# themattinthehatt/behavenet

Measured on AMD Instinct MI355X. Metric: AE training frames/sec (128x128x1, batch 256), higher is better.
Workload: dtype f32; 1 GPU; configs[1]: conv AE default arch, 1x128x128 f32 frames resident in HBM, 12 latents, batch 256 (chunks 200+56), fwd+bwd+Adam(amsgrad)

## Files before the change

behavenet_amd/csrc/conv_mfma_up.hip:

```cpp
#include <stdlib.h>
#include "bn_common.h"
#include "bn_fast.h"
#ifndef UP2_ST_AUX
#define UP2_ST_AUX 2
#endif
#ifndef UP2_ST_AUX_D
#define UP2_ST_AUX_D UP2_ST_AUX
#endif


typedef float floatx16 __attribute__((ext_vector_type(16)));

#define MF_THREADS 256
#define MF_MAX_LDS (64 * 1024)

static inline int ilog2_exact_up(int v) {
    int l = 0;
    while ((1 << l) < v) ++l;
    return ((1 << l) == v) ? l : -1;
}

struct UpTile {
    int F, AT_H, lgW, lgATW;
    int SWp, FS, CHS;
    int tiles_per_frame;
    int xl_floats;
};

template <int MR, int CC>
__global__ __launch_bounds__(MF_THREADS, 2) void k_up_mfma(
    const float* __restrict__ small, const float* __restrict__ w, const float* __restrict__ bias,
    float* __restrict__ out, const float* __restrict__ dact_src, BnGeom g, UpTile t, int act,
    int dact, float slope) {
    extern __shared__ __attribute__((aligned(16))) float smem[];
    float* xl = smem;
    float* wl = smem + t.xl_floats;
    constexpr int RS = 25;
    constexpr int TM = 32 * MR;
    constexpr int WCH = TM * RS;
    constexpr int WGRP = CC * WCH / 4;
    constexpr int WDMA = (WGRP + MF_THREADS - 1) / MF_THREADS;
    constexpr int WBUF = ((WDMA * MF_THREADS * 4) + 3) & ~3;
    const int tid = threadIdx.x, lane = tid & 63;
    const int wv = __builtin_amdgcn_readfirstlane(tid >> 6);
    const int li = lane & 31, kk = lane >> 5;

    const int grp = blockIdx.x / t.tiles_per_frame;
    const int rowt = blockIdx.x - grp * t.tiles_per_frame;
    const int n0 = grp * t.F;
    const int a0 = rowt * t.AT_H;
    const int m0 = blockIdx.y * TM;
    const int Ws = g.Ws, HWs = g.Hs * g.Ws;

    const int pos = 32 * wv + li;
    const int pf = pos >> t.lgATW;
    const int prem = pos & ((1 << t.lgATW) - 1);
    const int aj = prem >> t.lgW, bj = prem & (Ws - 1);
    const int base = pf * t.FS + (aj + 1) * t.SWp + (bj + 1) + kk * t.CHS;
    const bool pvalid = (n0 + pf) < g.N;

    int ioff = -2;
    if (tid < t.CHS) {
        const int f = tid / t.FS;
        const int r2 = tid - f * t.FS;
        const int y = r2 / t.SWp;
        const int x = r2 - y * t.SWp;
        const int p = a0 - 1 + y, q = x - 1;
        const bool ok = (n0 + f < g.N) && p >= 0 && p < g.Hs && q >= 0 && q < g.Ws;
        ioff = ok ? f * (g.Cs * HWs) + p * Ws + q : -1;
    }

    floatx16 acc[MR][4];
#pragma unroll
    for (int mr = 0; mr < MR; ++mr)
#pragma unroll
        for (int cl = 0; cl < 4; ++cl)
#pragma unroll
            for (int e = 0; e < 16; ++e) acc[mr][cl][e] = 0.f;

    float xr[CC];
    const __amdgpu_buffer_rsrc_t rs_w = __builtin_amdgcn_make_buffer_rsrc(
        (void*)w, 0, (int)((size_t)g.Cs * g.Cb * RS * 4), 0x00020000);

    auto issue_loads = [&](int c0, int buf) {
#pragma unroll
        for (int cc = 0; cc < CC; ++cc) {
            const int c = min(c0 + cc, g.Cs - 1);
            xr[cc] = small[((size_t)n0 * g.Cs + c) * HWs + max(ioff, 0)];
        }
#pragma unroll
        for (int k = 0; k < WDMA; ++k) {
            const int e = tid + MF_THREADS * k;
            const int cc = e / (WCH / 4);
            const int within = e - cc * (WCH / 4);
            const bool ok = (e < WGRP) && (c0 + cc < g.Cs);
            const int off = (((c0 + cc) * g.Cb + m0) * RS + 4 * within) * 4;
            __builtin_amdgcn_raw_ptr_buffer_load_lds(
                rs_w, wl + buf * WBUF + 4 * (MF_THREADS * k + 64 * wv), 16, ok ? off : 0x7fffffff,
                0, 0, 0);
        }
    };

    int cur = 0;
    issue_loads(0, 0);
    for (int c0 = 0; c0 < g.Cs; c0 += CC) {
        __syncthreads();
#pragma unroll
        for (int cc = 0; cc < CC; ++cc) {
            const bool cok = c0 + cc < g.Cs;
            if (ioff != -2) xl[cc * t.CHS + tid] = (cok && ioff >= 0) ? xr[cc] : 0.f;
        }
        asm volatile("s_waitcnt vmcnt(0)" ::: "memory");
        __syncthreads();
        if (c0 + CC < g.Cs) issue_loads(c0 + CC, cur ^ 1);
        const float* wcur = wl + cur * WBUF;

#pragma unroll 1
        for (int cp = 0; cp < CC / 2; ++cp) {
            const float* xb = xl + (2 * cp) * t.CHS + base;
            const float* wa = wcur + ((2 * cp + kk) * TM + li) * RS;
            float bv[3][3];
#pragma unroll
            for (int dy = 0; dy < 3; ++dy)
#pragma unroll
                for (int dx = 0; dx < 3; ++dx) bv[dy][dx] = xb[(dy - 1) * t.SWp + (dx - 1)];
#pragma unroll
            for (int rho = 0; rho < 2; ++rho) {
#pragma unroll
                for (int u = 0; u < 3; ++u) {
                    const int r = ((rho + 1) & 1) + 2 * u;
                    if (r >= 5) continue;
                    const int dy = ((rho + 1) >> 1) - u + 1;
#pragma unroll
                    for (int sig = 0; sig < 2; ++sig) {
#pragma unroll
                        for (int v = 0; v < 3; ++v) {
                            const int s = ((sig + 1) & 1) + 2 * v;
                            if (s >= 5) continue;
                            const int dx = ((sig + 1) >> 1) - v + 1;
#pragma unroll
                            for (int mr = 0; mr < MR; ++mr) {
                                const float av = wa[mr * 32 * RS + r * 5 + s];
                                acc[mr][rho * 2 + sig] = __builtin_amdgcn_mfma_f32_32x32x2f32(
                                    av, bv[dy][dx], acc[mr][rho * 2 + sig], 0, 0, 0);
                            }
                        }
                    }
                }
            }
        }
        cur ^= 1;
    }

    if (!pvalid) return;
    const int n = n0 + pf;
    const int Wb = g.Wb, HWb = g.Hb * g.Wb;
    const int h0 = 2 * (a0 + aj), w0 = 2 * bj;
#pragma unroll
    for (int mr = 0; mr < MR; ++mr) {
#pragma unroll
        for (int e = 0; e < 16; ++e) {
            const int m = m0 + mr * 32 + (e & 3) + 8 * (e >> 2) + 4 * kk;
            if (m >= g.Cb) continue;
            const float bm = bias ? bias[m] : 0.f;
#pragma unroll
            for (int rho = 0; rho < 2; ++rho) {
                const size_t idx = ((size_t)n * g.Cb + m) * HWb + (size_t)(h0 + rho) * Wb + w0;
                float2 v;
                v.x = bn_apply_act(acc[mr][rho * 2 + 0][e] + bm, act, slope);
                v.y = bn_apply_act(acc[mr][rho * 2 + 1][e] + bm, act, slope);
                if (dact_src) {
                    const float2 d = *reinterpret_cast<const float2*>(dact_src + idx);
                    v.x *= bn_act_grad_from_output(d.x, dact, slope);
                    v.y *= bn_act_grad_from_output(d.y, dact, slope);
                }
                *reinterpret_cast<float2*>(out + idx) = v;
            }
        }
    }
}

#define UP2_STR2(x) #x
#define UP2_STR(x) UP2_STR2(x)
#ifndef UP2_LOOP_ALIGN
#define UP2_LOOP_ALIGN 8
#endif
#ifndef UP2_LOOP_SHIFT
#define UP2_LOOP_SHIFT 32
#endif
#ifndef UP2_WGS
#define UP2_WGS 2
#endif
template <int LGW>
struct UP2 {
    static constexpr int Ws = 1 << LGW, HW = Ws * Ws, TP = 128;
    static constexpr int F = HW >= TP ? 1 : TP / HW;
    static constexpr int AT_H = HW >= TP ? TP / Ws : Ws;
    static constexpr int lgATW = (HW >= TP) ? 7 : 2 * LGW;
    static constexpr int SWp = Ws + 2, FS = (AT_H + 2) * SWp, CHS = F * FS;
    static constexpr int CHSP = (CHS + 63) / 64 * 64;
    static constexpr int TPF = (F == 1) ? Ws / AT_H : 1;
};

template <>
struct UP2<0> {
    static constexpr int CHSP = 256;
};
template <>
struct UP2<1> {
    static constexpr int CHSP = 320;
};
struct Up2Geo {
    int F, AT_H, ATW;
    int SWp, FS, CHS;
    int UPF;
};

__device__ __forceinline__ void up_dma16(__amdgpu_buffer_rsrc_t rsrc, float* lds, int voffset, int soffset) {
    __builtin_amdgcn_raw_ptr_buffer_load_lds(rsrc, lds, 16, voffset, soffset, 0, 0);
}
__device__ __forceinline__ void up_dma4(__amdgpu_buffer_rsrc_t rsrc, float* lds, int voffset, int soffset) {
    __builtin_amdgcn_raw_ptr_buffer_load_lds(rsrc, lds, 4, voffset, soffset, 0, 0);
}

template <int KV>
__device__ __forceinline__ constexpr bool up2_tap_live(int r, int s) {
    return r >= KV / 10 && r < KV % 10 && s >= KV / 10 && s < KV % 10;
}

template <int LGW, int CC, int KV>
__global__ __launch_bounds__(MF_THREADS, UP2_WGS) void k_up2_mfma(
    const float* __restrict__ small, const float* __restrict__ w, const float* __restrict__ bias,
    float* __restrict__ out, const float* __restrict__ dact_src, BnGeom g, int act, int dact,
    float slope, int cper, size_t zstride, Up2Geo tg) {
    extern __shared__ __attribute__((aligned(16))) float smem[];
    using T = UP2<LGW>;
    constexpr bool RT = LGW <= 1;
    const int c_beg = blockIdx.z * cper;
    const int c_end = min(g.Cs, c_beg + cper);
    out += blockIdx.z * zstride;
    constexpr int RS = 25, TM = 32;
    const int Ws = RT ? g.Ws : (1 << LGW), HWs = RT ? g.Hs * g.Ws : (1 << (2 * LGW)), SWp = RT ? tg.SWp : Ws + 2;
    constexpr int XBUF = CC * T::CHSP;
    constexpr int WCH = TM * RS;
    constexpr int WGRP = CC * WCH / 4;
    constexpr int WDMA = (WGRP + MF_THREADS - 1) / MF_THREADS;
    constexpr int WBUF = WDMA * MF_THREADS * 4;
    constexpr int XW = T::CHSP > MF_THREADS ? MF_THREADS / 64 : T::CHSP / 64;
    constexpr int OOB = 0x7fffffff;
    const int tid = threadIdx.x, lane = tid & 63;
    const int wv = __builtin_amdgcn_readfirstlane(tid >> 6);
    const int li = lane & 31, kk = lane >> 5;

    int grp, rowt, n0, a0, pf, aj, bj, tFS, tCHS;
    bool pvalid;
    const int m0 = blockIdx.y * TM;
    int u0 = 0, lidx = 0;
    if constexpr (RT) {
        grp = rowt = 0;
        u0 = blockIdx.x * tg.F;
        n0 = u0 / tg.UPF;
        int pos = 32 * wv + li;
        const bool inside = pos < tg.F * tg.ATW;
        if (!inside) pos = 0;
        const int uf = pos / tg.ATW;
        const int prem = pos - uf * tg.ATW;
        const int un = (u0 + uf) / tg.UPF;
        a0 = (u0 + uf - un * tg.UPF) * tg.AT_H;
        aj = prem / Ws;
        bj = prem - aj * Ws;
        pvalid = inside && un < g.N && (a0 + aj) < g.Hs;
        pf = un - n0;
        tFS = tg.FS; tCHS = tg.CHS;
        lidx = uf;
    } else {
        grp = blockIdx.x / T::TPF;
        rowt = blockIdx.x - grp * T::TPF;
        n0 = grp * T::F;
        a0 = rowt * T::AT_H;
        const int pos = 32 * wv + li;
        pf = pos >> T::lgATW;
        const int prem = pos & ((1 << T::lgATW) - 1);
        aj = prem >> LGW; bj = prem & (Ws - 1);
        pvalid = (n0 + pf) < g.N;
        tFS = T::FS; tCHS = T::CHS;
        lidx = pf;
    }
    const int Hs_rt = RT ? g.Hs : Ws;

    const __amdgpu_buffer_rsrc_t rs_x = __builtin_amdgcn_make_buffer_rsrc(
        (void*)small, 0, (int)((size_t)g.N * g.Cs * HWs * 4), 0x00020000);
    const __amdgpu_buffer_rsrc_t rs_w = __builtin_amdgcn_make_buffer_rsrc(
        (void*)w, 0, (int)((size_t)g.Cs * g.Cb * RS * 4), 0x00020000);
    auto tile_elem = [&](const int el) {
        if (el >= tCHS) return OOB;
        const int f = el / tFS, r2 = el - f * tFS;
        const int y = r2 / SWp, x = r2 - y * SWp;
        int fn = f, fa0 = a0;
        if constexpr (RT) {
            const int un = (u0 + f) / tg.UPF;
            fn = un - n0;
            fa0 = (u0 + f - un * tg.UPF) * tg.AT_H;
        }
        const int p = fa0 - 1 + y, q = x - 1;
        const bool ok = (n0 + fn < g.N) && p >= 0 && p < Hs_rt && q >= 0 && q < Ws;
        return ok ? (fn * (g.Cs * HWs) + p * Ws + q) * 4 : OOB;
    };
    const int xvo = tile_elem(tid);
    constexpr int NX2 = T::CHSP > MF_THREADS ? CC : 0;
    int xvo2 = OOB;
    if constexpr (NX2 > 0) xvo2 = tile_elem(tid + MF_THREADS);
    int wvo[WDMA];
#pragma unroll
    for (int k = 0; k < WDMA; ++k) {
        const int e = tid + MF_THREADS * k;
        const int cc = e / (WCH / 4), within = e - cc * (WCH / 4);
        wvo[k] = (e < WGRP) ? ((cc * g.Cb + m0) * RS + 4 * within) * 4 : OOB;
    }
    auto issue_dma = [&](const int d, const int buf, const int c0) __attribute__((always_inline)) {
        if (d < CC) {
            if (wv < XW)
                up_dma4(rs_x, smem + buf * XBUF + d * T::CHSP + 64 * wv, xvo,
                        (n0 * g.Cs + c0 + d) * HWs * 4);
        } else if (d < CC + NX2) {
            if (wv == 0 && tCHS > MF_THREADS)
                up_dma4(rs_x, smem + buf * XBUF + (d - CC) * T::CHSP + MF_THREADS, xvo2,
                        (n0 * g.Cs + c0 + d - CC) * HWs * 4);
        } else {
            const int k = d - CC - NX2;
            up_dma16(rs_w, smem + 2 * XBUF + buf * WBUF + 4 * (MF_THREADS * k + 64 * wv), wvo[k],
                     c0 * g.Cb * RS * 4);
        }
    };
    constexpr int NDMA = CC + NX2 + WDMA;

    floatx16 acc[4];
#pragma unroll
    for (int cl = 0; cl < 4; ++cl)
#pragma unroll
        for (int e = 0; e < 16; ++e) acc[cl][e] = 0.f;

    int xb_cur = (lidx * tFS + (aj + 1) * SWp + (bj + 1) + kk * T::CHSP) * 4;
    int xb_oth = xb_cur + XBUF * 4;
    int wa_cur = (2 * XBUF + (kk * TM + li) * RS) * 4;
    int wa_oth = wa_cur + WBUF * 4;
    asm volatile("" : "+v"(xb_cur)); asm volatile("" : "+v"(xb_oth));
    asm volatile("" : "+v"(wa_cur)); asm volatile("" : "+v"(wa_oth));
    int xu_cur = xb_cur - SWp * 4, xd_cur = xb_cur + SWp * 4;
    int xu_oth = xb_oth - SWp * 4, xd_oth = xb_oth + SWp * 4;
    if constexpr (RT) {
        asm volatile("" : "+v"(xu_cur)); asm volatile("" : "+v"(xd_cur));
        asm volatile("" : "+v"(xu_oth)); asm volatile("" : "+v"(xd_oth));
    }
    const char* sm = reinterpret_cast<const char*>(smem);

    struct Tap { int r, s, dy, dx, cl; };
    auto tap_of = [](const int j) {
        int n = 0;
        Tap tp = {0, 0, 0, 0, 0};
        for (int rho = 0; rho < 2; ++rho)
            for (int u = 0; u < 3; ++u) {
                const int r = ((rho + 1) & 1) + 2 * u;
                if (r >= 5) continue;
                for (int sig = 0; sig < 2; ++sig)
                    for (int v = 0; v < 3; ++v) {
                        const int s = ((sig + 1) & 1) + 2 * v;
                        if (s >= 5) continue;
                        if (n == j) tp = Tap{r, s, ((rho + 1) >> 1) - u + 1, ((sig + 1) >> 1) - v + 1, rho * 2 + sig};
                        ++n;
                    }
            }
        return tp;
    };
    constexpr int ORDER[25] = {12, 10, 13, 2, 14, 11, 17, 3, 18, 15, 19, 4, 0, 22, 16, 7, 1, 23, 20, 8, 5, 24, 21, 9, 6};
    auto load_a = [&](const int wa, const int cp, const int jj, float (&a)[25]) __attribute__((always_inline)) {
        const int j = ORDER[jj];
        const Tap tp = tap_of(j);
        a[j] = *reinterpret_cast<const float*>(sm + wa + ((2 * cp) * TM * RS + tp.r * 5 + tp.s) * 4);
    };
    auto load_b = [&](const int xb, const int xu, const int xd, const int cp, const int i, float (&b)[9]) __attribute__((always_inline)) {
        const int dy = i / 3, dx = i - 3 * dy;
        if constexpr (RT) {
            const int xr = dy == 0 ? xu : dy == 1 ? xb : xd;
            b[i] = *reinterpret_cast<const float*>(sm + xr + ((2 * cp) * T::CHSP + (dx - 1)) * 4);
        } else {
            constexpr int SW = (1 << LGW) + 2;
            b[i] = *reinterpret_cast<const float*>(sm + xb + ((2 * cp) * T::CHSP + (dy - 1) * SW + (dx - 1)) * 4);
        }
    };
    auto chunk_body = [&](const int xb, const int xu, const int xd, const int wa, const int nbuf, const bool more, const int c0n) __attribute__((always_inline)) {
        float av[25], bv[2][9];
#pragma unroll
        for (int i = 0; i < 9; ++i) load_b(xb, xu, xd, 0, i, bv[0]);
#pragma unroll
        for (int j = 0; j < 25; ++j) {
            const Tap t0 = tap_of(ORDER[j]);
            if (up2_tap_live<KV>(t0.r, t0.s)) load_a(wa, 0, j, av);
        }
#pragma unroll
        for (int cp = 0; cp < CC / 2; ++cp) {
#pragma unroll
            for (int j = 0; j < 25; ++j) {
                const Tap tp = tap_of(ORDER[j]);
                const bool live = up2_tap_live<KV>(tp.r, tp.s);
                if (live)
                    acc[tp.cl] = __builtin_amdgcn_mfma_f32_32x32x2f32(av[ORDER[j]], bv[cp & 1][tp.dy * 3 + tp.dx],
                                                                      acc[tp.cl], 0, 0, 0);
                if (cp + 1 < CC / 2) {
                    if (live) load_a(wa, cp + 1, j, av);
                    if (j >= 8 && j < 17) load_b(xb, xu, xd, cp + 1, j - 8, bv[(cp + 1) & 1]);
                }
                if (more && cp * 25 + j >= 2 && cp * 25 + j < 2 + NDMA) issue_dma(cp * 25 + j - 2, nbuf, c0n);
                __builtin_amdgcn_sched_barrier(0);
            }
        }
    };

    static_assert(NDMA + 2 <= (CC / 2) * 25, "DMA slots");
#pragma unroll
    for (int d = 0; d < NDMA; ++d) issue_dma(d, 0, c_beg);
    int cur = 0;
#ifdef UP2_LOOP_ALIGN
    asm volatile(".p2align " UP2_STR(UP2_LOOP_ALIGN) "\n .rept " UP2_STR(UP2_LOOP_SHIFT) "\n s_nop 0\n .endr" ::: "memory");
#endif
    for (int c0 = c_beg; c0 < c_end; c0 += CC) {
        asm volatile("s_waitcnt vmcnt(0)" ::: "memory");
        __syncthreads();
        chunk_body(xb_cur, xu_cur, xd_cur, wa_cur, cur ^ 1, c0 + CC < c_end, c0 + CC);
        cur ^= 1;
        int tmp = xb_cur; xb_cur = xb_oth; xb_oth = tmp;
        tmp = wa_cur; wa_cur = wa_oth; wa_oth = tmp;
        if constexpr (RT) {
            tmp = xu_cur; xu_cur = xu_oth; xu_oth = tmp;
            tmp = xd_cur; xd_cur = xd_oth; xd_oth = tmp;
        }
    }

    const int Wb = g.Wb, HWb = g.Hb * g.Wb;
    const int obytes = (int)((size_t)g.N * g.Cb * HWb * 4);
    const __amdgpu_buffer_rsrc_t ro = __builtin_amdgcn_make_buffer_rsrc((void*)out, 0, obytes, 0x00020000);
    const __amdgpu_buffer_rsrc_t rd = __builtin_amdgcn_make_buffer_rsrc(
        (void*)dact_src, 0, dact_src ? obytes : 0, 0x00020000);
    const __amdgpu_buffer_rsrc_t rbs = __builtin_amdgcn_make_buffer_rsrc(
        (void*)bias, 0, bias ? g.Cb * 4 : 0, 0x00020000);
    const int mlane = m0 + 4 * kk;
    const int n = n0 + pf;
    const int vo = pvalid ? (int)((((size_t)n * g.Cb + mlane) * HWb + (size_t)(2 * (a0 + aj)) * Wb + 2 * bj) * 4) : OOB;
    typedef float floatx2u __attribute__((ext_vector_type(2)));
    typedef unsigned int uintx2u __attribute__((ext_vector_type(2)));
    if (act != BN_ACT_SIGMOID && dact != BN_ACT_SIGMOID) {
        const float es = (act == BN_ACT_LRELU) ? slope : 1.f;
        const float ds = (dact == BN_ACT_LRELU) ? slope : 1.f;
        float bz[16];
#pragma unroll
        for (int e = 0; e < 16; ++e)
            bz[e] = __builtin_bit_cast(float, __builtin_amdgcn_raw_buffer_load_b32(
                rbs, (mlane + (e & 3) + 8 * (e >> 2)) * 4, 0, 0));
#pragma unroll
        for (int rho = 0; rho < 2; ++rho) {
            floatx2u d[16];
            if (dact_src) {
#pragma unroll
                for (int e = 0; e < 16; ++e) {
                    const int mo = (e & 3) + 8 * (e >> 2);
                    d[e] = __builtin_bit_cast(floatx2u, __builtin_amdgcn_raw_buffer_load_b64(
                        rd, (mlane + mo < g.Cb) ? vo : OOB, (mo * HWb + rho * Wb) * 4, 0));
                }
            }
#pragma unroll
            for (int e = 0; e < 16; ++e) {
                const int mo = (e & 3) + 8 * (e >> 2);
                floatx2u v;
                v.x = acc[rho * 2 + 0][e] + bz[e];
                v.y = acc[rho * 2 + 1][e] + bz[e];
                v.x = v.x > 0.f ? v.x : v.x * es;
                v.y = v.y > 0.f ? v.y : v.y * es;
                if (dact_src) {
                    v.x *= d[e].x > 0.f ? 1.f : ds;
                    v.y *= d[e].y > 0.f ? 1.f : ds;
                }
                if (UP2_ST_AUX_D != UP2_ST_AUX && dact_src)
                    __builtin_amdgcn_raw_buffer_store_b64(__builtin_bit_cast(uintx2u, v), ro,
                                                          (mlane + mo < g.Cb) ? vo : OOB,
                                                          (mo * HWb + rho * Wb) * 4, UP2_ST_AUX_D);
                else
                    __builtin_amdgcn_raw_buffer_store_b64(__builtin_bit_cast(uintx2u, v), ro,
                                                          (mlane + mo < g.Cb) ? vo : OOB,
                                                          (mo * HWb + rho * Wb) * 4, UP2_ST_AUX);
            }
        }
    } else {
        if (!pvalid) return;
        const int h0 = 2 * (a0 + aj), w0 = 2 * bj;
#pragma unroll
        for (int e = 0; e < 16; ++e) {
            const int m = m0 + (e & 3) + 8 * (e >> 2) + 4 * kk;
            if (m >= g.Cb) continue;
            const float bm = bias ? bias[m] : 0.f;
#pragma unroll
            for (int rho = 0; rho < 2; ++rho) {
                const size_t idx = ((size_t)n * g.Cb + m) * HWb + (size_t)(h0 + rho) * Wb + w0;
                float2 v;
                v.x = bn_apply_act(acc[rho * 2 + 0][e] + bm, act, slope);
                v.y = bn_apply_act(acc[rho * 2 + 1][e] + bm, act, slope);
                if (dact_src) {
                    const float2 d = *reinterpret_cast<const float2*>(dact_src + idx);
                    v.x *= bn_act_grad_from_output(d.x, dact, slope);
                    v.y *= bn_act_grad_from_output(d.y, dact, slope);
                }
                *reinterpret_cast<float2*>(out + idx) = v;
            }
        }
    }
}

static size_t up_lds_bytes(int xl_floats, int MR, int CC) {
    const int wgrp = CC * 32 * MR * 25 / 4;
    const int wdma = (wgrp + MF_THREADS - 1) / MF_THREADS;
    return ((size_t)xl_floats + 2 * (size_t)wdma * MF_THREADS * 4) * 4;
}

static bool up_tile(const BnGeom& g, int MR, int CC, UpTile* t, int* n_wg) {
    const int TP = 128;
    const int lgW = ilog2_exact_up(g.Ws), lgH = ilog2_exact_up(g.Hs);
    if (lgW < 0 || lgH < 0) return false;
    if (g.Hb != 2 * g.Hs || g.Wb != 2 * g.Ws) return false;
    const int HW = g.Hs * g.Ws;
    if (g.Ws > TP) return false;
    if (HW >= TP) {
        t->F = 1;
        t->AT_H = TP / g.Ws;
    } else {
        t->F = TP / HW;
        t->AT_H = g.Hs;
    }
    t->lgW = lgW;
    t->lgATW = ilog2_exact_up(t->AT_H * g.Ws);
    t->SWp = g.Ws + 2;
    t->FS = (t->AT_H + 2) * t->SWp;
    t->CHS = t->F * t->FS;
    if (t->CHS > MF_THREADS) return false;
    t->tiles_per_frame = (t->F == 1) ? g.Hs / t->AT_H : 1;
    t->xl_floats = (CC * t->CHS + 3) & ~3;
    const size_t lds = up_lds_bytes(t->xl_floats, MR, CC);
    if (lds > MF_MAX_LDS) return false;
    if ((g.Cb & 3) != 0) return false;
    if ((size_t)g.Cs * g.Cb * 25 * 4 >= 0x7fffffffull) return false;
    const int groups = (g.N + t->F - 1) / t->F;
    *n_wg = groups * t->tiles_per_frame * ((g.Cb + 32 * MR - 1) / (32 * MR));
    return true;
}

static bool up2_ok(const BnGeom& g) {
    const int lgw = ilog2_exact_up(g.Ws);
    if (g.Hs != g.Ws || lgw < 3 || lgw > 5) return false;
    if ((g.Cs % 4) != 0 || (g.Cb & 3) != 0) return false;
    if ((size_t)g.N * g.Cb * g.Hb * g.Wb * 4 >= 0x7fffffffull) return false;
    if ((size_t)g.N * g.Cs * g.Hs * g.Ws * 4 >= 0x7fffffffull) return false;
    return true;
}

static int up2_splits(const BnGeom& g, int lgw, int cc) {
    const int F = (1 << (2 * lgw)) >= 128 ? 1 : 128 >> (2 * lgw);
    const int tpf = (1 << (2 * lgw)) >= 128 ? (1 << (2 * lgw)) / 128 : 1;
    const int wgs = ((g.N + F - 1) / F) * tpf * ((g.Cb + 31) / 32);
    if (wgs > 128) return 1;
    int s = 256 / wgs;
    while (s > 1 && (g.Cs % (s * cc) != 0 || g.Cs / s < 32)) --s;
    return s > 8 ? 8 : (s < 1 ? 1 : s);
}

template <int LGW, int CC, int KV>
static int launch_up2(const float* small, const float* w, const float* bias, float* out,
                      const float* dact_src, const BnGeom& g, int act, int dact, float slope,
                      hipStream_t st, int splits, void* ws) {
    using T = UP2<LGW>;
    constexpr int WDMA = (CC * 32 * 25 / 4 + MF_THREADS - 1) / MF_THREADS;
    constexpr size_t lds = ((size_t)2 * CC * T::CHSP + (size_t)2 * WDMA * MF_THREADS * 4) * 4;
    static bool attr_set = false;
    if (!attr_set) {
        hipError_t e = hipFuncSetAttribute((const void*)k_up2_mfma<LGW, CC, KV>,
                                           hipFuncAttributeMaxDynamicSharedMemorySize, (int)lds);
        if (e != hipSuccess) return (int)e;
        attr_set = true;
    }
    const int groups = (g.N + T::F - 1) / T::F;
    dim3 grid(groups * T::TPF, (g.Cb + 31) / 32, splits);
    if (splits > 1) {
        if (!ws) return BN_E_WORKSPACE;
        const size_t total = (size_t)g.N * g.Cb * g.Hb * g.Wb;
        BN_LAUNCH_MAIN((k_up2_mfma<LGW, CC, KV>), grid, dim3(MF_THREADS), lds, st, small, w,
                       (const float*)nullptr, (float*)ws, (const float*)nullptr, g, BN_ACT_NONE,
                       BN_ACT_NONE, slope, g.Cs / splits, total, Up2Geo{});
        BN_LAUNCH_CHECK();
        return bn_launch_split_epilogue((const float*)ws, bias, out, dact_src, total, splits, g.Cb,
                                        g.Hb * g.Wb, act, dact, slope, st);
    }
    BN_LAUNCH_MAIN((k_up2_mfma<LGW, CC, KV>), grid, dim3(MF_THREADS), lds, st, small, w, bias, out,
                       dact_src, g, act, dact, slope, g.Cs, (size_t)0, Up2Geo{});
    BN_LAUNCH_CHECK();
    return 0;
}

static bool up2g_geo_lim(const BnGeom& g, Up2Geo* t, int chsp, float* fill_out);
static bool up2g_geo(const BnGeom& g, Up2Geo* t) {
    float f0 = 0.f, f1 = 0.f;
    Up2Geo t1;
    const bool ok0 = up2g_geo_lim(g, t, UP2<0>::CHSP, &f0);
    const bool ok1 = ok0 && up2g_geo_lim(g, &t1, UP2<1>::CHSP, &f1);
    if (ok1 && f1 > 1.1f * f0) { *t = t1; return true; }
    return ok0;
}
static bool up2g_geo_lim(const BnGeom& g, Up2Geo* t, int chsp, float* fill_out) {
    if (g.R != 5 || g.S != 5 || g.stride != 2 || g.pt != 1 || g.pl != 1) return false;
    if (g.Hb != 2 * g.Hs || g.Wb != 2 * g.Ws) return false;
    if ((g.Cs % 4) != 0 || (g.Cb & 3) != 0 || g.Cb < 16) return false;
    if ((size_t)g.N * g.Cb * g.Hb * g.Wb * 4 >= 0x7fffffffull) return false;
    if ((size_t)g.N * g.Cs * g.Hs * g.Ws * 4 >= 0x7fffffffull) return false;
    if ((size_t)g.Cs * g.Cb * 25 * 4 >= 0x7fffffffull) return false;
    const int TP = 128, HW = g.Hs * g.Ws;
    if (g.Ws < 2 || g.Ws > TP) return false;
    t->SWp = g.Ws + 2;
    (void)HW;
    float best = 0.f;
    int b_upf = 0, b_ath = 0, b_F = 0;
    for (int upf = 1; upf <= g.Hs; ++upf) {
        const int ath = (g.Hs + upf - 1) / upf;
        if ((g.Hs + ath - 1) / ath != upf || ath * g.Ws > TP) continue;
        int F = TP / (ath * g.Ws);
        const int fs = (ath + 2) * t->SWp;
        while (F >= 1 && F * fs > chsp) --F;
        if (F < 1) continue;
        const float fill = (float)(F * ath * g.Ws) / (float)TP * (float)g.Hs / (float)(upf * ath);
        if (fill > best + 1e-6f) { best = fill; b_upf = upf; b_ath = ath; b_F = F; }
        if (best >= 0.999f) break;
    }
    if (b_upf == 0) return false;
    *fill_out = best;
    t->UPF = b_upf; t->AT_H = b_ath; t->F = b_F;
    t->FS = (b_ath + 2) * t->SWp;
    t->CHS = b_F * t->FS;
    t->ATW = t->AT_H * g.Ws;
    return true;
}

static int up2g_splits(const BnGeom& g, const Up2Geo& t, int cc) {
    const int wgs = ((g.N * t.UPF + t.F - 1) / t.F) * ((g.Cb + 31) / 32);
    if (wgs > 128) return 1;
    int s = 256 / wgs;
    while (s > 1 && (g.Cs % (s * cc) != 0 || g.Cs / s < 32)) --s;
    return s > 8 ? 8 : (s < 1 ? 1 : s);
}

template <int KV, int LG>
static int launch_up2g_img(const float* small, const float* w, const float* bias, float* out,
                       const float* dact_src, const BnGeom& g, int act, int dact, float slope,
                       hipStream_t st, int splits, void* ws) {
    constexpr int CC = 4;
    Up2Geo t;
    if (!up2g_geo(g, &t)) return BN_E_SHAPE;
    constexpr int WDMA = (CC * 32 * 25 / 4 + MF_THREADS - 1) / MF_THREADS;
    constexpr size_t lds = ((size_t)2 * CC * UP2<LG>::CHSP + (size_t)2 * WDMA * MF_THREADS * 4) * 4;
    static bool attr_set = false;
    if (!attr_set) {
        hipError_t e = hipFuncSetAttribute((const void*)k_up2_mfma<LG, CC, KV>,
                                           hipFuncAttributeMaxDynamicSharedMemorySize, (int)lds);
        if (e != hipSuccess) return (int)e;
        attr_set = true;
    }
    dim3 grid((g.N * t.UPF + t.F - 1) / t.F, (g.Cb + 31) / 32, splits);
    if (splits > 1) {
        if (!ws) return BN_E_WORKSPACE;
        const size_t total = (size_t)g.N * g.Cb * g.Hb * g.Wb;
        BN_LAUNCH_MAIN((k_up2_mfma<LG, CC, KV>), grid, dim3(MF_THREADS), lds, st, small, w,
                       (const float*)nullptr, (float*)ws, (const float*)nullptr, g, BN_ACT_NONE,
                       BN_ACT_NONE, slope, g.Cs / splits, total, t);
        BN_LAUNCH_CHECK();
        return bn_launch_split_epilogue((const float*)ws, bias, out, dact_src, total, splits, g.Cb,
                                        g.Hb * g.Wb, act, dact, slope, st);
    }
    BN_LAUNCH_MAIN((k_up2_mfma<LG, CC, KV>), grid, dim3(MF_THREADS), lds, st, small, w, bias, out,
                       dact_src, g, act, dact, slope, g.Cs, (size_t)0, t);
    BN_LAUNCH_CHECK();
    return 0;
}

template <int KV>
static int launch_up2g(const float* small, const float* w, const float* bias, float* out,
                       const float* dact_src, const BnGeom& g, int act, int dact, float slope,
                       hipStream_t st, int splits, void* ws) {
    Up2Geo t;
    if (!up2g_geo(g, &t)) return BN_E_SHAPE;
    return t.CHS > UP2<0>::CHSP
        ? launch_up2g_img<KV, 1>(small, w, bias, out, dact_src, g, act, dact, slope, st, splits, ws)
        : launch_up2g_img<KV, 0>(small, w, bias, out, dact_src, g, act, dact, slope, st, splits, ws);
}

BnFastPlan bn_fast_up_plan(const BnGeom& g) {
    BnFastPlan p = {false, "k_up_generic", 0, 0, 0, 0, 0, 0};
    if (g.R != 5 || g.S != 5 || g.stride != 2 || g.pt != 1 || g.pl != 1) return p;
    if (g.Cb < 16 || g.Cs < 2) return p;
    UpTile t;
    int nwg2 = 0, nwg1 = 0;
    const bool ok2 = g.Cb >= 64 && up_tile(g, 2, 4, &t, &nwg2);
    const bool ok1 = up_tile(g, 1, 4, &t, &nwg1);
    if (!ok1 && !ok2) {
        Up2Geo tg;
        if (!up2g_geo(g, &tg)) return p;
        p.supported = true;
        p.a = 1; p.c = 4; p.variant = 3;
        p.kernel_name = tg.CHS > UP2<0>::CHSP ? "k_up2_mfma<1, 4>" : "k_up2_mfma<0, 4>";
        p.d = up2g_splits(g, tg, 4);
        p.ws_bytes = p.d > 1 ? (size_t)p.d * g.N * g.Cb * g.Hb * g.Wb * sizeof(float) : 0;
        return p;
    }
    p.supported = true;
    p.a = (ok2 && (nwg2 >= 768 || !ok1)) ? 2 : 1;
    p.c = 4;
    p.kernel_name = p.a == 2 ? "k_up_mfma<2, 4>" : "k_up_mfma<1, 4>";
    if ((p.a == 1 || ok1) && up2_ok(g)) {
        p.a = 1;
        p.variant = 2;
        const int lgw = ilog2_exact_up(g.Ws);
        static const char* const n4[6] = {"", "", "", "k_up2_mfma<3, 4>", "k_up2_mfma<4, 4>", "k_up2_mfma<5, 4>"};
        p.kernel_name = n4[lgw];
        p.d = up2_splits(g, lgw, p.c);
        p.ws_bytes = p.d > 1 ? (size_t)p.d * g.N * g.Cb * g.Hb * g.Wb * sizeof(float) : 0;
    }
    return p;
}

int bn_launch_up_fast(const BnFastPlan& plan, const float* small, const float* w,
                      const float* bias, float* out, const float* dact_src, const BnGeom& g,
                      int act, int dact, float slope, void* ws, hipStream_t st) {
    const int MR = plan.a, CC = plan.c;
    if (plan.variant == 3)
        return g.KV == 4 && g.K0 == 1
            ? launch_up2g<14>(small, w, bias, out, dact_src, g, act, dact, slope, st, plan.d > 1 ? plan.d : 1, ws)
            : g.KV == 4
            ? launch_up2g<4>(small, w, bias, out, dact_src, g, act, dact, slope, st, plan.d > 1 ? plan.d : 1, ws)
            : launch_up2g<5>(small, w, bias, out, dact_src, g, act, dact, slope, st, plan.d > 1 ? plan.d : 1, ws);
    if (plan.variant == 2) {
        const int lgw = ilog2_exact_up(g.Ws);
        const int splits = plan.d > 1 ? plan.d : 1;
#define UP2_CASE(L, C)                                                                          \
    if (lgw == L && CC == C)                                                                    \
        return launch_up2<L, C, 5>(small, w, bias, out, dact_src, g, act, dact, slope, st, splits, ws);
#define UP2_CASE4(L)                                                                            \
    if (lgw == L && CC == 4 && g.KV == 4 && g.K0 == 1)                                          \
        return launch_up2<L, 4, 14>(small, w, bias, out, dact_src, g, act, dact, slope, st, splits, ws); \
    if (lgw == L && CC == 4 && g.KV == 4)                                                       \
        return launch_up2<L, 4, 4>(small, w, bias, out, dact_src, g, act, dact, slope, st, splits, ws);
        UP2_CASE4(3) UP2_CASE4(4) UP2_CASE4(5)
#undef UP2_CASE4
        UP2_CASE(3, 4) UP2_CASE(4, 4) UP2_CASE(5, 4)
#undef UP2_CASE
        return BN_E_SHAPE;
    }
    UpTile t;
    int nwg = 0;
    if (!up_tile(g, MR, CC, &t, &nwg)) return BN_E_SHAPE;
    const int groups = (g.N + t.F - 1) / t.F;
    dim3 grid(groups * t.tiles_per_frame, (g.Cb + 32 * MR - 1) / (32 * MR));
    const size_t lds = up_lds_bytes(t.xl_floats, MR, CC);
    if (MR == 2) {
        BN_LAUNCH_MAIN((k_up_mfma<2, 4>), grid, dim3(MF_THREADS), lds, st, small, w, bias, out,
                           dact_src, g, t, act, dact, slope);
    } else {
        BN_LAUNCH_MAIN((k_up_mfma<1, 4>), grid, dim3(MF_THREADS), lds, st, small, w, bias, out,
                           dact_src, g, t, act, dact, slope);
    }
    BN_LAUNCH_CHECK();
    return 0;
}
```

Measured before the change: 58950 frames/s.

## Make up-conv MFMA kernel persistent with cross-tile DMA prefetch

Turns the stride-2 transposed-conv MFMA kernel into a persistent kernel for the fixed-tile path. A grid sized to CU count times workgroups per CU walks flattened (channel-block, spatial) units, and the first chunk of the next unit's input and weights is prefetched during the last chunk of the current one. The goal is to cut per-workgroup launch and prologue cost and hide the DMA latency at tile boundaries. LDS is padded to a fixed size so exactly two workgroups fit per CU. This adds per-unit address setup, an epilogue inside the loop, and less dynamic load balancing.

```diff
diff --git a/behavenet_amd/csrc/conv_mfma_up.hip b/behavenet_amd/csrc/conv_mfma_up.hip
--- a/behavenet_amd/csrc/conv_mfma_up.hip
+++ b/behavenet_amd/csrc/conv_mfma_up.hip
@@ -1,4 +1,5 @@
 #include <stdlib.h>
+#include <atomic>
 #include "bn_common.h"
 #include "bn_fast.h"
 #ifndef UP2_ST_AUX
@@ -13,6 +14,7 @@
 
 #define MF_THREADS 256
 #define MF_MAX_LDS (64 * 1024)
+#define BN_UP2_MAX_DEVICES 64
 
 static inline int ilog2_exact_up(int v) {
     int l = 0;
@@ -191,6 +193,11 @@
 #ifndef UP2_WGS
 #define UP2_WGS 2
 #endif
+#define UP2_CU_LDS_BYTES (160 * 1024)
+#ifndef UP2_LDS_BYTES
+#define UP2_LDS_BYTES (56 * 1024)
+#endif
+static_assert(3 * UP2_LDS_BYTES > UP2_CU_LDS_BYTES && 2 * UP2_LDS_BYTES <= UP2_CU_LDS_BYTES, "two workgroups per CU");
 template <int LGW>
 struct UP2 {
     static constexpr int Ws = 1 << LGW, HW = Ws * Ws, TP = 128;
@@ -232,7 +239,7 @@
 __global__ __launch_bounds__(MF_THREADS, UP2_WGS) void k_up2_mfma(
     const float* __restrict__ small, const float* __restrict__ w, const float* __restrict__ bias,
     float* __restrict__ out, const float* __restrict__ dact_src, BnGeom g, int act, int dact,
-    float slope, int cper, size_t zstride, Up2Geo tg) {
+    float slope, int cper, size_t zstride, Up2Geo tg, int nx) {
     extern __shared__ __attribute__((aligned(16))) float smem[];
     using T = UP2<LGW>;
     constexpr bool RT = LGW <= 1;
@@ -252,93 +259,114 @@
     const int wv = __builtin_amdgcn_readfirstlane(tid >> 6);
     const int li = lane & 31, kk = lane >> 5;
 
-    int grp, rowt, n0, a0, pf, aj, bj, tFS, tCHS;
-    bool pvalid;
-    const int m0 = blockIdx.y * TM;
-    int u0 = 0, lidx = 0;
+    int pf = 0, aj, bj, lidx;
+    bool inside = true;
+    int tFS, tCHS;
     if constexpr (RT) {
-        grp = rowt = 0;
-        u0 = blockIdx.x * tg.F;
-        n0 = u0 / tg.UPF;
+        tFS = tg.FS; tCHS = tg.CHS;
         int pos = 32 * wv + li;
-        const bool inside = pos < tg.F * tg.ATW;
+        inside = pos < tg.F * tg.ATW;
         if (!inside) pos = 0;
-        const int uf = pos / tg.ATW;
-        const int prem = pos - uf * tg.ATW;
-        const int un = (u0 + uf) / tg.UPF;
-        a0 = (u0 + uf - un * tg.UPF) * tg.AT_H;
+        lidx = pos / tg.ATW;
+        const int prem = pos - lidx * tg.ATW;
         aj = prem / Ws;
         bj = prem - aj * Ws;
-        pvalid = inside && un < g.N && (a0 + aj) < g.Hs;
-        pf = un - n0;
-        tFS = tg.FS; tCHS = tg.CHS;
-        lidx = uf;
     } else {
-        grp = blockIdx.x / T::TPF;
-        rowt = blockIdx.x - grp * T::TPF;
-        n0 = grp * T::F;
-        a0 = rowt * T::AT_H;
+        tFS = T::FS; tCHS = T::CHS;
         const int pos = 32 * wv + li;
         pf = pos >> T::lgATW;
         const int prem = pos & ((1 << T::lgATW) - 1);
         aj = prem >> LGW; bj = prem & (Ws - 1);
-        pvalid = (n0 + pf) < g.N;
-        tFS = T::FS; tCHS = T::CHS;
         lidx = pf;
     }
     const int Hs_rt = RT ? g.Hs : Ws;
+
+    const int nunits = nx * ((g.Cb + TM - 1) / TM);
+    struct Unit { int m0, n0, a0, u0; };
+    auto unit_of = [&](const int unit) {
+        Unit q;
+        const int by = unit / nx, bx = unit - by * nx;
+        q.m0 = by * TM;
+        if constexpr (RT) {
+            q.u0 = bx * tg.F;
+            q.n0 = q.u0 / tg.UPF;
+            q.a0 = 0;
+        } else {
+            const int grp = bx / T::TPF;
+            q.u0 = 0;
+            q.n0 = grp * T::F;
+            q.a0 = (bx - grp * T::TPF) * T::AT_H;
+        }
+        return q;
+    };
 
     const __amdgpu_buffer_rsrc_t rs_x = __builtin_amdgcn_make_buffer_rsrc(
         (void*)small, 0, (int)((size_t)g.N * g.Cs * HWs * 4), 0x00020000);
     const __amdgpu_buffer_rsrc_t rs_w = __builtin_amdgcn_make_buffer_rsrc(
         (void*)w, 0, (int)((size_t)g.Cs * g.Cb * RS * 4), 0x00020000);
-    auto tile_elem = [&](const int el) {
+    auto tile_elem = [&](const int el, const Unit& q) {
         if (el >= tCHS) return OOB;
         const int f = el / tFS, r2 = el - f * tFS;
         const int y = r2 / SWp, x = r2 - y * SWp;
-        int fn = f, fa0 = a0;
+        int fn = f, fa0 = q.a0;
         if constexpr (RT) {
-            const int un = (u0 + f) / tg.UPF;
-            fn = un - n0;
-            fa0 = (u0 + f - un * tg.UPF) * tg.AT_H;
-        }
-        const int p = fa0 - 1 + y, q = x - 1;
-        const bool ok = (n0 + fn < g.N) && p >= 0 && p < Hs_rt && q >= 0 && q < Ws;
-        return ok ? (fn * (g.Cs * HWs) + p * Ws + q) * 4 : OOB;
-    };
-    const int xvo = tile_elem(tid);
+            const int un = (q.u0 + f) / tg.UPF;
+            fn = un - q.n0;
+            fa0 = (q.u0 + f - un * tg.UPF) * tg.AT_H;
+        }
+        const int p = fa0 - 1 + y, c = x - 1;
+        const bool ok = (q.n0 + fn < g.N) && p >= 0 && p < Hs_rt && c >= 0 && c < Ws;
+        return ok ? (fn * (g.Cs * HWs) + p * Ws + c) * 4 : OOB;
+    };
     constexpr int NX2 = T::CHSP > MF_THREADS ? CC : 0;
-    int xvo2 = OOB;
-    if constexpr (NX2 > 0) xvo2 = tile_elem(tid + MF_THREADS);
-    int wvo[WDMA];
-#pragma unroll
-    for (int k = 0; k < WDMA; ++k) {
-        const int e = tid + MF_THREADS * k;
-        const int cc = e / (WCH / 4), within = e - cc * (WCH / 4);
-        wvo[k] = (e < WGRP) ? ((cc * g.Cb + m0) * RS + 4 * within) * 4 : OOB;
-    }
+    int d_n0 = 0, d_xvo = OOB, d_xvo2 = OOB;
+    int d_wvo[WDMA];
+    auto dma_setup = [&](const int unit) {
+        const Unit q = unit_of(unit);
+        d_n0 = q.n0;
+        d_xvo = tile_elem(tid, q);
+        if constexpr (NX2 > 0) d_xvo2 = tile_elem(tid + MF_THREADS, q);
+#pragma unroll
+        for (int k = 0; k < WDMA; ++k) {
+            const int e = tid + MF_THREADS * k;
+            const int cc = e / (WCH / 4), within = e - cc * (WCH / 4);
+            d_wvo[k] = (e < WGRP) ? ((cc * g.Cb + q.m0) * RS + 4 * within) * 4 : OOB;
+        }
+    };
+    int o_m0 = 0, o_n = 0, o_row = 0;
+    bool o_valid = false;
+    auto out_setup = [&](const int unit) {
+        const Unit q = unit_of(unit);
+        o_m0 = q.m0;
+        if constexpr (RT) {
+            const int un = (q.u0 + lidx) / tg.UPF;
+            o_n = un;
+            o_row = (q.u0 + lidx - un * tg.UPF) * tg.AT_H + aj;
+            o_valid = inside && un < g.N && o_row < g.Hs;
+        } else {
+            o_n = q.n0 + pf;
+            o_row = q.a0 + aj;
+            o_valid = o_n < g.N;
+        }
+    };
     auto issue_dma = [&](const int d, const int buf, const int c0) __attribute__((always_inline)) {
         if (d < CC) {
             if (wv < XW)
-                up_dma4(rs_x, smem + buf * XBUF + d * T::CHSP + 64 * wv, xvo,
-                        (n0 * g.Cs + c0 + d) * HWs * 4);
+                up_dma4(rs_x, smem + buf * XBUF + d * T::CHSP + 64 * wv, d_xvo,
+                        (d_n0 * g.Cs + c0 + d) * HWs * 4);
         } else if (d < CC + NX2) {
             if (wv == 0 && tCHS > MF_THREADS)
-                up_dma4(rs_x, smem + buf * XBUF + (d - CC) * T::CHSP + MF_THREADS, xvo2,
-                        (n0 * g.Cs + c0 + d - CC) * HWs * 4);
+                up_dma4(rs_x, smem + buf * XBUF + (d - CC) * T::CHSP + MF_THREADS, d_xvo2,
+                        (d_n0 * g.Cs + c0 + d - CC) * HWs * 4);
         } else {
             const int k = d - CC - NX2;
-            up_dma16(rs_w, smem + 2 * XBUF + buf * WBUF + 4 * (MF_THREADS * k + 64 * wv), wvo[k],
+            up_dma16(rs_w, smem + 2 * XBUF + buf * WBUF + 4 * (MF_THREADS * k + 64 * wv), d_wvo[k],
                      c0 * g.Cb * RS * 4);
         }
     };
     constexpr int NDMA = CC + NX2 + WDMA;
 
     floatx16 acc[4];
-#pragma unroll
-    for (int cl = 0; cl < 4; ++cl)
-#pragma unroll
-        for (int e = 0; e < 16; ++e) acc[cl][e] = 0.f;
 
     int xb_cur = (lidx * tFS + (aj + 1) * SWp + (bj + 1) + kk * T::CHSP) * 4;
     int xb_oth = xb_cur + XBUF * 4;
@@ -417,25 +445,6 @@
     };
 
     static_assert(NDMA + 2 <= (CC / 2) * 25, "DMA slots");
-#pragma unroll
-    for (int d = 0; d < NDMA; ++d) issue_dma(d, 0, c_beg);
-    int cur = 0;
-#ifdef UP2_LOOP_ALIGN
-    asm volatile(".p2align " UP2_STR(UP2_LOOP_ALIGN) "\n .rept " UP2_STR(UP2_LOOP_SHIFT) "\n s_nop 0\n .endr" ::: "memory");
-#endif
-    for (int c0 = c_beg; c0 < c_end; c0 += CC) {
-        asm volatile("s_waitcnt vmcnt(0)" ::: "memory");
-        __syncthreads();
-        chunk_body(xb_cur, xu_cur, xd_cur, wa_cur, cur ^ 1, c0 + CC < c_end, c0 + CC);
-        cur ^= 1;
-        int tmp = xb_cur; xb_cur = xb_oth; xb_oth = tmp;
-        tmp = wa_cur; wa_cur = wa_oth; wa_oth = tmp;
-        if constexpr (RT) {
-            tmp = xu_cur; xu_cur = xu_oth; xu_oth = tmp;
-            tmp = xd_cur; xd_cur = xd_oth; xd_oth = tmp;
-        }
-    }
-
     const int Wb = g.Wb, HWb = g.Hb * g.Wb;
     const int obytes = (int)((size_t)g.N * g.Cb * HWb * 4);
     const __amdgpu_buffer_rsrc_t ro = __builtin_amdgcn_make_buffer_rsrc((void*)out, 0, obytes, 0x00020000);
@@ -443,74 +452,112 @@
         (void*)dact_src, 0, dact_src ? obytes : 0, 0x00020000);
     const __amdgpu_buffer_rsrc_t rbs = __builtin_amdgcn_make_buffer_rsrc(
         (void*)bias, 0, bias ? g.Cb * 4 : 0, 0x00020000);
-    const int mlane = m0 + 4 * kk;
-    const int n = n0 + pf;
-    const int vo = pvalid ? (int)((((size_t)n * g.Cb + mlane) * HWb + (size_t)(2 * (a0 + aj)) * Wb + 2 * bj) * 4) : OOB;
     typedef float floatx2u __attribute__((ext_vector_type(2)));
     typedef unsigned int uintx2u __attribute__((ext_vector_type(2)));
-    if (act != BN_ACT_SIGMOID && dact != BN_ACT_SIGMOID) {
-        const float es = (act == BN_ACT_LRELU) ? slope : 1.f;
-        const float ds = (dact == BN_ACT_LRELU) ? slope : 1.f;
-        float bz[16];
-#pragma unroll
-        for (int e = 0; e < 16; ++e)
-            bz[e] = __builtin_bit_cast(float, __builtin_amdgcn_raw_buffer_load_b32(
-                rbs, (mlane + (e & 3) + 8 * (e >> 2)) * 4, 0, 0));
-#pragma unroll
-        for (int rho = 0; rho < 2; ++rho) {
-            floatx2u d[16];
-            if (dact_src) {
+
+    int cur = 0;
+    auto chunk = [&](const bool more, const int c0n) __attribute__((always_inline)) {
+        asm volatile("s_waitcnt vmcnt(0)" ::: "memory");
+        __syncthreads();
+        chunk_body(xb_cur, xu_cur, xd_cur, wa_cur, cur ^ 1, more, c0n);
+        cur ^= 1;
+        int tmp = xb_cur; xb_cur = xb_oth; xb_oth = tmp;
+        tmp = wa_cur; wa_cur = wa_oth; wa_oth = tmp;
+        if constexpr (RT) {
+            tmp = xu_cur; xu_cur = xu_oth; xu_oth = tmp;
+            tmp = xd_cur; xd_cur = xd_oth; xd_oth = tmp;
+        }
+    };
+
+    int unit = blockIdx.x;
+    dma_setup(unit);
+#pragma unroll
+    for (int d = 0; d < NDMA; ++d) issue_dma(d, 0, c_beg);
+    for (;;) {
+        acc[0] = acc[1] = acc[2] = acc[3] = (floatx16)(0.f);
+        out_setup(unit);
+        const int unit_next = unit + gridDim.x;
+        const bool walk_on = !RT && unit_next < nunits;
+#ifdef UP2_LOOP_ALIGN
+        asm volatile(".p2align " UP2_STR(UP2_LOOP_ALIGN) "\n .rept " UP2_STR(UP2_LOOP_SHIFT) "\n s_nop 0\n .endr" ::: "memory");
+#endif
+        if constexpr (RT) {
+            for (int c0 = c_beg; c0 < c_end; c0 += CC) chunk(c0 + CC < c_end, c0 + CC);
+        } else {
+            for (int c0 = c_beg; c0 + CC < c_end; c0 += CC) chunk(true, c0 + CC);
+            if (walk_on) dma_setup(unit_next);
+            chunk(walk_on, c_beg);
+        }
+
+        const int m0 = o_m0, n = o_n;
+        const bool pvalid = o_valid;
+        const int mlane = m0 + 4 * kk;
+        const int vo = pvalid ? (int)((((size_t)n * g.Cb + mlane) * HWb + (size_t)(2 * o_row) * Wb + 2 * bj) * 4) : OOB;
+        if (act != BN_ACT_SIGMOID && dact != BN_ACT_SIGMOID) {
+            const float es = (act == BN_ACT_LRELU) ? slope : 1.f;
+            const float ds = (dact == BN_ACT_LRELU) ? slope : 1.f;
+            float bz[16];
+#pragma unroll
+            for (int e = 0; e < 16; ++e)
+                bz[e] = __builtin_bit_cast(float, __builtin_amdgcn_raw_buffer_load_b32(
+                    rbs, (mlane + (e & 3) + 8 * (e >> 2)) * 4, 0, 0));
+#pragma unroll
+            for (int rho = 0; rho < 2; ++rho) {
+                floatx2u d[16];
+                if (dact_src) {
+#pragma unroll
+                    for (int e = 0; e < 16; ++e) {
+                        const int mo = (e & 3) + 8 * (e >> 2);
+                        d[e] = __builtin_bit_cast(floatx2u, __builtin_amdgcn_raw_buffer_load_b64(
+                            rd, (mlane + mo < g.Cb) ? vo : OOB, (mo * HWb + rho * Wb) * 4, 0));
+                    }
+                }
 #pragma unroll
                 for (int e = 0; e < 16; ++e) {
                     const int mo = (e & 3) + 8 * (e >> 2);
-                    d[e] = __builtin_bit_cast(floatx2u, __builtin_amdgcn_raw_buffer_load_b64(
-                        rd, (mlane + mo < g.Cb) ? vo : OOB, (mo * HWb + rho * Wb) * 4, 0));
+                    floatx2u v;
+                    v.x = acc[rho * 2 + 0][e] + bz[e];
+                    v.y = acc[rho * 2 + 1][e] + bz[e];
+                    v.x = v.x > 0.f ? v.x : v.x * es;
+                    v.y = v.y > 0.f ? v.y : v.y * es;
+                    if (dact_src) {
+                        v.x *= d[e].x > 0.f ? 1.f : ds;
+                        v.y *= d[e].y > 0.f ? 1.f : ds;
+                    }
+                    if (UP2_ST_AUX_D != UP2_ST_AUX && dact_src)
+                        __builtin_amdgcn_raw_buffer_store_b64(__builtin_bit_cast(uintx2u, v), ro,
+                                                              (mlane + mo < g.Cb) ? vo : OOB,
+                                                              (mo * HWb + rho * Wb) * 4, UP2_ST_AUX_D);
+                    else
+                        __builtin_amdgcn_raw_buffer_store_b64(__builtin_bit_cast(uintx2u, v), ro,
+                                                              (mlane + mo < g.Cb) ? vo : OOB,
+                                                              (mo * HWb + rho * Wb) * 4, UP2_ST_AUX);
                 }
             }
+        } else {
+            const int h0 = 2 * o_row, w0 = 2 * bj;
 #pragma unroll
             for (int e = 0; e < 16; ++e) {
-                const int mo = (e & 3) + 8 * (e >> 2);
-                floatx2u v;
-                v.x = acc[rho * 2 + 0][e] + bz[e];
-                v.y = acc[rho * 2 + 1][e] + bz[e];
-                v.x = v.x > 0.f ? v.x : v.x * es;
-                v.y = v.y > 0.f ? v.y : v.y * es;
-                if (dact_src) {
-                    v.x *= d[e].x > 0.f ? 1.f : ds;
-                    v.y *= d[e].y > 0.f ? 1.f : ds;
+                const int m = m0 + (e & 3) + 8 * (e >> 2) + 4 * kk;
+                if (!pvalid || m >= g.Cb) continue;
+                const float bm = bias ? bias[m] : 0.f;
+#pragma unroll
+                for (int rho = 0; rho < 2; ++rho) {
+                    const size_t idx = ((size_t)n * g.Cb + m) * HWb + (size_t)(h0 + rho) * Wb + w0;
+                    float2 v;
+                    v.x = bn_apply_act(acc[rho * 2 + 0][e] + bm, act, slope);
+                    v.y = bn_apply_act(acc[rho * 2 + 1][e] + bm, act, slope);
+                    if (dact_src) {
+                        const float2 d = *reinterpret_cast<const float2*>(dact_src + idx);
+                        v.x *= bn_act_grad_from_output(d.x, dact, slope);
+                        v.y *= bn_act_grad_from_output(d.y, dact, slope);
+                    }
+                    *reinterpret_cast<float2*>(out + idx) = v;
                 }
-                if (UP2_ST_AUX_D != UP2_ST_AUX && dact_src)
-                    __builtin_amdgcn_raw_buffer_store_b64(__builtin_bit_cast(uintx2u, v), ro,
-                                                          (mlane + mo < g.Cb) ? vo : OOB,
-                                                          (mo * HWb + rho * Wb) * 4, UP2_ST_AUX_D);
-                else
-                    __builtin_amdgcn_raw_buffer_store_b64(__builtin_bit_cast(uintx2u, v), ro,
-                                                          (mlane + mo < g.Cb) ? vo : OOB,
-                                                          (mo * HWb + rho * Wb) * 4, UP2_ST_AUX);
             }
         }
-    } else {
-        if (!pvalid) return;
-        const int h0 = 2 * (a0 + aj), w0 = 2 * bj;
-#pragma unroll
-        for (int e = 0; e < 16; ++e) {
-            const int m = m0 + (e & 3) + 8 * (e >> 2) + 4 * kk;
-            if (m >= g.Cb) continue;
-            const float bm = bias ? bias[m] : 0.f;
-#pragma unroll
-            for (int rho = 0; rho < 2; ++rho) {
-                const size_t idx = ((size_t)n * g.Cb + m) * HWb + (size_t)(h0 + rho) * Wb + w0;
-                float2 v;
-                v.x = bn_apply_act(acc[rho * 2 + 0][e] + bm, act, slope);
-                v.y = bn_apply_act(acc[rho * 2 + 1][e] + bm, act, slope);
-                if (dact_src) {
-                    const float2 d = *reinterpret_cast<const float2*>(dact_src + idx);
-                    v.x *= bn_act_grad_from_output(d.x, dact, slope);
-                    v.y *= bn_act_grad_from_output(d.y, dact, slope);
-                }
-                *reinterpret_cast<float2*>(out + idx) = v;
-            }
-        }
+        if (!walk_on) break;
+        unit = unit_next;
     }
 }
 
@@ -570,13 +617,32 @@
     return s > 8 ? 8 : (s < 1 ? 1 : s);
 }
 
+static int up2_grid(int units, int splits, dim3* grid) {
+    static std::atomic<int> slots_of[BN_UP2_MAX_DEVICES];
+    int dev = 0;
+    hipError_t e = hipGetDevice(&dev);
+    if (e != hipSuccess) return (int)e;
+    int slots = (dev >= 0 && dev < BN_UP2_MAX_DEVICES) ? slots_of[dev].load(std::memory_order_relaxed) : 0;
+    if (slots == 0) {
+        int cus = 0;
+        e = hipDeviceGetAttribute(&cus, hipDeviceAttributeMultiprocessorCount, dev);
+        if (e != hipSuccess) return (int)e;
+        if (cus < 1) return BN_E_SHAPE;
+        slots = (UP2_CU_LDS_BYTES / UP2_LDS_BYTES) * cus;
+        if (dev >= 0 && dev < BN_UP2_MAX_DEVICES) slots_of[dev].store(slots, std::memory_order_relaxed);
+    }
+    *grid = dim3((splits == 1 && units > slots) ? slots : units, 1, splits);
+    return 0;
+}
+
 template <int LGW, int CC, int KV>
 static int launch_up2(const float* small, const float* w, const float* bias, float* out,
                       const float* dact_src, const BnGeom& g, int act, int dact, float slope,
                       hipStream_t st, int splits, void* ws) {
     using T = UP2<LGW>;
     constexpr int WDMA = (CC * 32 * 25 / 4 + MF_THREADS - 1) / MF_THREADS;
-    constexpr size_t lds = ((size_t)2 * CC * T::CHSP + (size_t)2 * WDMA * MF_THREADS * 4) * 4;
+    static_assert(((size_t)2 * CC * T::CHSP + (size_t)2 * WDMA * MF_THREADS * 4) * 4 <= UP2_LDS_BYTES, "LDS images");
+    constexpr size_t lds = UP2_LDS_BYTES;
     static bool attr_set = false;
     if (!attr_set) {
         hipError_t e = hipFuncSetAttribute((const void*)k_up2_mfma<LGW, CC, KV>,
@@ -585,19 +651,22 @@
         attr_set = true;
     }
     const int groups = (g.N + T::F - 1) / T::F;
-    dim3 grid(groups * T::TPF, (g.Cb + 31) / 32, splits);
+    const int nx = groups * T::TPF;
+    dim3 grid;
+    const int rc = up2_grid(nx * ((g.Cb + 31) / 32), splits, &grid);
+    if (rc != 0) return rc;
     if (splits > 1) {
         if (!ws) return BN_E_WORKSPACE;
         const size_t total = (size_t)g.N * g.Cb * g.Hb * g.Wb;
         BN_LAUNCH_MAIN((k_up2_mfma<LGW, CC, KV>), grid, dim3(MF_THREADS), lds, st, small, w,
                        (const float*)nullptr, (float*)ws, (const float*)nullptr, g, BN_ACT_NONE,
-                       BN_ACT_NONE, slope, g.Cs / splits, total, Up2Geo{});
+                       BN_ACT_NONE, slope, g.Cs / splits, total, Up2Geo{}, nx);
         BN_LAUNCH_CHECK();
         return bn_launch_split_epilogue((const float*)ws, bias, out, dact_src, total, splits, g.Cb,
                                         g.Hb * g.Wb, act, dact, slope, st);
     }
     BN_LAUNCH_MAIN((k_up2_mfma<LGW, CC, KV>), grid, dim3(MF_THREADS), lds, st, small, w, bias, out,
-                       dact_src, g, act, dact, slope, g.Cs, (size_t)0, Up2Geo{});
+                       dact_src, g, act, dact, slope, g.Cs, (size_t)0, Up2Geo{}, nx);
     BN_LAUNCH_CHECK();
     return 0;
 }
@@ -668,19 +737,20 @@
         if (e != hipSuccess) return (int)e;
         attr_set = true;
     }
-    dim3 grid((g.N * t.UPF + t.F - 1) / t.F, (g.Cb + 31) / 32, splits);
+    const int nx = (g.N * t.UPF + t.F - 1) / t.F;
+    dim3 grid(nx * ((g.Cb + 31) / 32), 1, splits);
     if (splits > 1) {
         if (!ws) return BN_E_WORKSPACE;
         const size_t total = (size_t)g.N * g.Cb * g.Hb * g.Wb;
         BN_LAUNCH_MAIN((k_up2_mfma<LG, CC, KV>), grid, dim3(MF_THREADS), lds, st, small, w,
                        (const float*)nullptr, (float*)ws, (const float*)nullptr, g, BN_ACT_NONE,
-                       BN_ACT_NONE, slope, g.Cs / splits, total, t);
+                       BN_ACT_NONE, slope, g.Cs / splits, total, t, nx);
         BN_LAUNCH_CHECK();
         return bn_launch_split_epilogue((const float*)ws, bias, out, dact_src, total, splits, g.Cb,
                                         g.Hb * g.Wb, act, dact, slope, st);
     }
     BN_LAUNCH_MAIN((k_up2_mfma<LG, CC, KV>), grid, dim3(MF_THREADS), lds, st, small, w, bias, out,
-                       dact_src, g, act, dact, slope, g.Cs, (size_t)0, t);
+                       dact_src, g, act, dact, slope, g.Cs, (size_t)0, t, nx);
     BN_LAUNCH_CHECK();
     return 0;
 }
```

Result: no change. 59420 frames/s, median of 6 (+0.8%).
